# boqian-li/ETCH

Hardware: AMD Instinct MI355X
Metric: scans/s (5k pts, eq-net + 50-iter SMPL fit) (higher is better)
Workload: dtype f32 (matrix operands: 2 x fp16 planes per fp32 value, fp32 accumulate)

## Files before the change

### etch_amd/csrc/gemm.hip

```cpp
#include "common.h"
#include "split_bf16.h"
#include <cstdlib>
#include <cstring>

typedef float f32x4 __attribute__((ext_vector_type(4)));

struct GemmArgs {
    int R, K, O;
    const float* X; long ldx; const int* row_idx; int grp, p_in, p_out;
    const float* W; long ldw;
    const float* bias; const float* scale; const float* shift;
    int act;
    const float* res; long ldr; int res_mode;
    float* Y; long ldy;
};

#define G_BM 64
#define G_BN 64
#define G_BK 32
#define G_LD 40

template <bool VEC>
__device__ __forceinline__ float4 ld4_guard(const float* row, int k, int K, bool row_ok) {
    float4 v = make_float4(0.f, 0.f, 0.f, 0.f);
// ... 261 lines not shown
    l = __float_as_uint(r - __uint_as_float(m & 0xffff0000u));
}
__device__ __forceinline__ void g_split8(const float4 v0, const float4 v1, g_bf16x8 (&o)[3]) {
    const float v[8] = {v0.x, v0.y, v0.z, v0.w, v1.x, v1.y, v1.z, v1.w};
    unsigned h[8], m[8], l[8];
#pragma unroll
    for (int i = 0; i < 8; ++i) g_split(v[i], h[i], m[i], l[i]);
    typedef unsigned u32x4 __attribute__((ext_vector_type(4)));
#define G_PK(a) (u32x4){__builtin_amdgcn_perm(a[1], a[0], 0x07060302u), __builtin_amdgcn_perm(a[3], a[2], 0x07060302u), \
                        __builtin_amdgcn_perm(a[5], a[4], 0x07060302u), __builtin_amdgcn_perm(a[7], a[6], 0x07060302u)}
    const u32x4 ph = G_PK(h), pm = G_PK(m), pl = G_PK(l);
#undef G_PK
    o[0] = __builtin_bit_cast(g_bf16x8, ph); o[1] = __builtin_bit_cast(g_bf16x8, pm); o[2] = __builtin_bit_cast(g_bf16x8, pl);
}

template <int K, int SPW, int RP, bool F16 = false>
__global__ void __launch_bounds__(512) gemm_ws_split_kernel(GemmArgs a, long rows_per_block) {
    constexpr int FD_ROWS = 64, SB = K + 8, KT = K / 32, PLANE = FD_ROWS * SB;
    constexpr int NPL = F16 ? 2 : 3;
    constexpr int SG = 8 / RP;
    constexpr int RTW = (FD_ROWS / 16) / RP;
    extern __shared__ __attribute__((aligned(16))) float lds[];
    unsigned short* Xp = reinterpret_cast<unsigned short*>(lds);
    float* rsc = lds + 2 * NPL * PLANE / 2;
    float* wtab = rsc + 2 * FD_ROWS;
    const int tid = threadIdx.x, lane = tid & 63, wave = __builtin_amdgcn_readfirstlane(tid >> 6);
    const int fr = lane & 15, fg = lane >> 4;
    const int sg = wave % SG, rp = wave / SG;
    g_bf16x8 wf[KT][SPW][NPL];
    float4 wk4[SPW];
    constexpr bool EPI_REGS = KT * SPW * 12 <= 96;
    float4 bs[EPI_REGS ? SPW : 1], sc[EPI_REGS ? SPW : 1], sh[EPI_REGS ? SPW : 1];
// ... 33 lines not shown
            }
        } else {
#pragma unroll
            for (int t = 0; t < KT; ++t) {
                const float* p = a.W + (long)(o + fr) * a.ldw + 32 * t + 8 * fg;
                g_bf16x8 q3[3];
                g_split8(*reinterpret_cast<const float4*>(p), *reinterpret_cast<const float4*>(p + 4), q3);
#pragma unroll
                for (int pl = 0; pl < NPL; ++pl) wf[t][s2][pl] = q3[pl % 3];
            }
        }
        if constexpr (EPI_REGS) epi_load(o, bs[s2], sc[s2], sh[s2]);
    }
    constexpr int C4 = K / 4;
    constexpr int XL = (FD_ROWS * C4 + 511) / 512;
    const long row_lo = (long)blockIdx.x * rows_per_block, row_hi = row_lo + rows_per_block < a.R ? row_lo + rows_per_block : a.R;
    float4 xn[XL];
    static_assert(512 % C4 == 0 && (FD_ROWS * C4) % 512 == 0, "tile staging assumes whole 512-element passes");
    constexpr int RSTEP = 512 / C4;
    const int row0 = tid / C4, c0 = (tid % C4) * 4;
    auto fetch = [&](long r0) {
        const float* src = a.X + (r0 + row0) * a.ldx + c0;
#pragma unroll
        for (int h = 0; h < XL; ++h) {
            xn[h] = make_float4(0.f, 0.f, 0.f, 0.f);
            if (r0 + row0 + h * RSTEP < row_hi) xn[h] = *reinterpret_cast<const float4*>(src + (long)(h * RSTEP) * a.ldx);
        }
    };
    auto stage = [&](unsigned short* P, float* rs) {
        unsigned short* d0 = P + row0 * SB + c0;
#pragma unroll
        for (int h = 0; h < XL; ++h) {
            if constexpr (F16) {
                const int kx = etch_scale_exp(etch_group_max<C4>(etch_max4abs(xn[h], 0.f)));
                const float sx = ldexpf(1.0f, kx);
                uint2 ph, pl;
// ... 46 lines not shown
                float4 v;
                if constexpr (F16) {
                    v = make_float4(fmaf(acc[s2][0], rsv * wk4[s2].x, b_.x), fmaf(acc[s2][1], rsv * wk4[s2].y, b_.y), fmaf(acc[s2][2], rsv * wk4[s2].z, b_.z),
                                    fmaf(acc[s2][3], rsv * wk4[s2].w, b_.w));
                } else {
                    v = make_float4(acc[s2][0] + b_.x, acc[s2][1] + b_.y, acc[s2][2] + b_.z, acc[s2][3] + b_.w);
                }
                if (a.scale) { v.x = v.x * s_.x + h_.x; v.y = v.y * s_.y + h_.y; v.z = v.z * s_.z + h_.z; v.w = v.w * s_.w + h_.w; }
                float4 rs = make_float4(0.f, 0.f, 0.f, 0.f);
                if (a.res_mode != 0) rs = *reinterpret_cast<const float4*>(a.res + r * a.ldr + o);
                if (a.res_mode == 1) { v.x += rs.x; v.y += rs.y; v.z += rs.z; v.w += rs.w; }
                if (a.act == 1) { v.x = fmaxf(v.x, 0.f); v.y = fmaxf(v.y, 0.f); v.z = fmaxf(v.z, 0.f); v.w = fmaxf(v.w, 0.f); }
                else if (a.act == 2) { v.x = v.x > 0.f ? v.x : 0.01f * v.x; v.y = v.y > 0.f ? v.y : 0.01f * v.y; v.z = v.z > 0.f ? v.z : 0.01f * v.z; v.w = v.w > 0.f ? v.w : 0.01f * v.w; }
                if (a.res_mode == 2) { v.x += rs.x; v.y += rs.y; v.z += rs.z; v.w += rs.w; }
                *reinterpret_cast<float4*>(a.Y + r * a.ldy + o) = v;
            }
        }
    };
    if (row_lo >= row_hi) return;
    fetch(row_lo);
    stage(Xp, rsc);
    fetch(row_lo + FD_ROWS);
    __syncthreads();
    if constexpr (F16) {
#pragma unroll
        for (int s2 = 0; s2 < SPW; ++s2) wk4[s2] = *reinterpret_cast<const float4*>(&wtab[(wave * SPW + s2) * 16 + 4 * fg]);
    }
    int buf = 0;
    for (long r0 = row_lo; r0 < row_hi; r0 += FD_ROWS, buf ^= 1) {
        const unsigned short* P = Xp + buf * NPL * PLANE;
        row_tile(P, rp * RTW, r0, rsc + buf * FD_ROWS);
        stage(Xp + (buf ^ 1) * NPL * PLANE, rsc + (buf ^ 1) * FD_ROWS);
        if constexpr (EPI_REGS) fetch(r0 + 2 * FD_ROWS);
#pragma unroll
        for (int i = 1; i < RTW; ++i) row_tile(P, rp * RTW + i, r0, rsc + buf * FD_ROWS);
        if constexpr (!EPI_REGS) fetch(r0 + 2 * FD_ROWS);
        __syncthreads();
    }
}

template <int K, int SPW, int RP, bool F16 = false>
static int launch_ws_split(const GemmArgs& a, hipStream_t st) {
    constexpr int FD_ROWS = 64;
    const size_t lds = (size_t)2 * (F16 ? 2 : 3) * FD_ROWS * (K + 8) * 2 + (size_t)2 * FD_ROWS * sizeof(float) + (size_t)8 * SPW * 16 * sizeof(float);
    auto kern = gemm_ws_split_kernel<K, SPW, RP, F16>;
    static int per_cu = 0;
    if (per_cu == 0) {
        if (lds > 64 * 1024) {
            hipError_t e = hipFuncSetAttribute((const void*)kern, hipFuncAttributeMaxDynamicSharedMemorySize, (int)lds);
            if (e != hipSuccess) return (int)e;
        }
        int n = 0;
        if (hipOccupancyMaxActiveBlocksPerMultiprocessor(&n, (const void*)kern, 512, lds) != hipSuccess || n < 1) n = 1;
        per_cu = n;
    }
    long nb = (long)etch_cu_count() * per_cu;
    long rpb = (a.R + nb - 1) / nb;
#ifndef GEMM_WS_MIN_TILES
#define GEMM_WS_MIN_TILES 4
#endif
    if (rpb < GEMM_WS_MIN_TILES * FD_ROWS) rpb = GEMM_WS_MIN_TILES * FD_ROWS;
    rpb = (rpb + FD_ROWS - 1) / FD_ROWS * FD_ROWS;
    nb = (a.R + rpb - 1) / rpb;
    hipLaunchKernelGGL(kern, dim3((unsigned)nb), dim3(512), lds, st, a, rpb);
    ETCH_RETURN_IF_LAUNCH_FAILED();
    return ETCH_OK;
}

extern "C" int etch_linear(int R, int K, int O, const float* X, long ldx, const int* row_idx, int grp, int p_in, int p_out,
                           const float* W, long ldw, const float* bias, const float* scale, const float* shift, int act,
                           const float* res, long ldr, int res_mode, float* Y, long ldy, void* stream) {
    if (R <= 0 || O <= 0) return ETCH_OK;
    if (K <= 0) return ETCH_EINVAL;
    if ((scale == nullptr) != (shift == nullptr)) return ETCH_EINVAL;
    if (res_mode != 0 && res == nullptr) return ETCH_EINVAL;
    if (row_idx && (grp <= 0 || p_out <= 0)) return ETCH_EINVAL;
    GemmArgs a{R, K, O, X, ldx, row_idx, grp, p_in, p_out, W, ldw, bias, scale, shift, act, res, ldr, res_mode, Y, ldy};
    const bool vx = !(K & 3) && !(ldx & 3) && !((uintptr_t)X & 15);
    const bool vw = !(K & 3) && !(ldw & 3) && !((uintptr_t)W & 15);
    hipStream_t st = (hipStream_t)stream;
    if (K == 1) {
// ... 32 lines not shown
```

### etch_amd/csrc/pt.hip

```cpp
#include "common.h"

struct PtAttnParams {
    const float* p;
    const float* xq; const float* xk; const float* xv; long ldq;
    const int* idx;
    const float* W0; const float* b0; const float* s_p; const float* t_p;
    const float* W3; const float* b3;
    const float* s_w0; const float* t_w0;
    const float* W2T; const float* b2;
    const float* s_w3; const float* t_w3;
    const float* W5; const float* b5;
    const float* s_out; const float* t_out;
    float* out; long ldo;
    int n, c, ns;
};

__global__ void __launch_bounds__(128) pt_attention_kernel(PtAttnParams a) {
    extern __shared__ __attribute__((aligned(16))) float sm[];
    const int c = a.c, ns = a.ns, cs = c >> 3;
    float* s_pr = sm;
    float* s_w = s_pr + ns * c;
    float* s_h = s_w + ns * c;
    float* s_l = s_h + ns * cs;
    float* s_p3 = s_l + ns * cs;
// ... 559 lines not shown
    return v;
}
template <int NS>
__device__ __forceinline__ float pt_group_max(float v) {
    v = fmaxf(v, pt_dpp<0xB1>(v));
    v = fmaxf(v, pt_dpp<0x4E>(v));
    v = fmaxf(v, pt_dpp<0x141>(v));
    if (NS == 16) v = fmaxf(v, pt_dpp<0x140>(v));
    return v;
}

#ifndef PT_MFMA_WGS
#define PT_MFMA_WGS 4
#endif
template <int C, int NS>
__global__ void __launch_bounds__(256, PT_MFMA_WGS) pt_attention_mfma_kernel(PtAttnParams a, const float* __restrict__ W2, long ntiles) {
    constexpr int CS = C / 8;
    constexpr int MT = CS <= 16 ? 1 : CS / 16;
    constexpr int KT = C / 16;
    constexpr int PPW = 16 / NS;
    constexpr bool W2_LDS = C <= 256;
    constexpr int LDW = C + 4;
    extern __shared__ __attribute__((aligned(16))) float cst[];
    float* W3s = cst;
    float* b3s = W3s + 3 * C;
    float* scs = b3s + C;
    float* shs = scs + C;
    float* sos = shs + C;
    float* tos = sos + C;
    float* b2s = tos + C;
    float* s3s = b2s + CS;
// ... 6 lines not shown
    for (int e = tid; e < C; e += 256) {
        b3s[e] = a.b3[e]; scs[e] = a.s_w0[e]; shs[e] = a.t_w0[e];
        sos[e] = a.s_out ? a.s_out[e] : 1.f; tos[e] = a.s_out ? a.t_out[e] : 0.f;
    }
    for (int e = tid; e < CS; e += 256) { b2s[e] = a.b2[e]; s3s[e] = a.s_w3[e]; t3s[e] = a.t_w3[e]; b5s[e] = a.b5[e]; }
    for (int e = tid; e < CS * CS; e += 256) W5s[e] = a.W5[e];
    if (W2_LDS)
        for (int e = tid; e < CS * C / 4; e += 256) {
            const int row = e / (C / 4), c4 = e - row * (C / 4);
            *reinterpret_cast<float4*>(&W2s[row * LDW + c4 * 4]) = *reinterpret_cast<const float4*>(W2 + (size_t)row * C + c4 * 4);
        }
    __syncthreads();
    const int lane = tid & 63, wave = tid >> 6;
    const int fr = lane & 15, fg = lane >> 4;
    const int pw = fr / NS, jn = fr % NS;
    for (long tile = blockIdx.x; tile < ntiles; tile += gridDim.x) {
    asm volatile("" ::: "memory");
    const long base = (tile * 4 + wave) * PPW;
    const bool valid = base + pw < a.n;
    const int i = valid ? (int)(base + pw) : a.n - 1;
    const int j = a.idx[(size_t)i * NS + jn];
    float h[3];
    pt_rel_hidden(a, i, j, h);
    const float* kr = a.xk + (size_t)j * a.ldq;
    const float* qr = a.xq + (size_t)i * a.ldq;
    const float* vr = a.xv + (size_t)j * a.ldq;

    pf32x4 acc[MT];
#pragma unroll
    for (int mt = 0; mt < MT; ++mt) acc[mt] = (pf32x4){0.f, 0.f, 0.f, 0.f};
#pragma unroll 4
    for (int t = 0; t < KT; ++t) {
        const int ch0 = t * 16 + fg * 4;
        const float4 k4 = *reinterpret_cast<const float4*>(kr + ch0), q4 = *reinterpret_cast<const float4*>(qr + ch0);
        const float4 wa = *reinterpret_cast<const float4*>(W3s + ch0 * 3), wb = *reinterpret_cast<const float4*>(W3s + ch0 * 3 + 4),
// ... 68 lines not shown
                if (jn == 0 && valid) {
                    if (a.s_out) {
                        const float4 so = *reinterpret_cast<const float4*>(sos + ch0), to = *reinterpret_cast<const float4*>(tos + ch0);
                        o0 = fmaxf(o0 * so.x + to.x, 0.f); o1 = fmaxf(o1 * so.y + to.y, 0.f);
                        o2 = fmaxf(o2 * so.z + to.z, 0.f); o3 = fmaxf(o3 * so.w + to.w, 0.f);
                    }
                    *reinterpret_cast<float4*>(orow + ch0) = make_float4(o0, o1, o2, o3);
                }
            }
        }
    }
    }
}

template <int C_, int NS_>
static int launch_pt_mfma(const PtAttnParams& a, const float* W2, hipStream_t st) {
    constexpr int CS = C_ / 8, PPW = 16 / NS_;
    const size_t lds = (size_t)(8 * C_ + 4 * CS + CS * CS + (C_ <= 256 ? CS * (C_ + 4) : 0)) * sizeof(float);
    auto kern = pt_attention_mfma_kernel<C_, NS_>;
    static int per_cu = 0;
    if (per_cu == 0) {
        if (lds > 64 * 1024 && hipFuncSetAttribute((const void*)kern, hipFuncAttributeMaxDynamicSharedMemorySize, (int)lds) != hipSuccess) return ETCH_EUNSUPPORTED;
        int nb = 0;
        if (hipOccupancyMaxActiveBlocksPerMultiprocessor(&nb, (const void*)kern, 256, lds) != hipSuccess || nb < 1) nb = 1;
        per_cu = nb > 8 ? 8 : nb;
    }
    const long ntiles = ((long)a.n + 4 * PPW - 1) / (4 * PPW);
    long blocks = (long)etch_cu_count() * per_cu;
    if (blocks > ntiles) blocks = ntiles;
    hipLaunchKernelGGL(kern, dim3((unsigned)blocks), dim3(256), lds, st, a, W2, ntiles);
    ETCH_RETURN_IF_LAUNCH_FAILED();
    return ETCH_OK;
}

extern "C" int etch_pt_attention_mfma(int n, int c, int ns, const float* p, const float* xq, const float* xk, const float* xv, long ldq,
                                      const int* idx, const float* const* params, const float* W2, float* out, long ldo, void* stream) {
    if (n <= 0) return ETCH_OK;
    if ((ldq & 3) || (ldo & 3) || !W2) return ETCH_EINVAL;
    PtAttnParams a;
    fill_pt_params(a, n, c, ns, p, xq, xk, xv, ldq, idx, params, out, ldo);
    hipStream_t st = (hipStream_t)stream;
#define PT_MFMA_CASE(C_, NS_) \
    if (c == C_ && ns == NS_) return launch_pt_mfma<C_, NS_>(a, W2, st);
    PT_MFMA_CASE(64, 8) PT_MFMA_CASE(128, 8) PT_MFMA_CASE(64, 16) PT_MFMA_CASE(128, 16) PT_MFMA_CASE(256, 16) PT_MFMA_CASE(512, 16)
#undef PT_MFMA_CASE
    return ETCH_EUNSUPPORTED;
}

__global__ void __launch_bounds__(256) pt_down_gather_max_kernel(int m, int ns, int co, const float* __restrict__ ux, long ldu,
                                                                 const float* __restrict__ p, const float* __restrict__ new_p,
                                                                 const int* __restrict__ idx, const float* __restrict__ Wp,
                                                                 const float* __restrict__ scale, const float* __restrict__ shift,
                                                                 float* __restrict__ out) {
    const int c4 = co >> 2;
    const size_t total = (size_t)m * c4;
    for (size_t e = (size_t)blockIdx.x * 256 + threadIdx.x; e < total; e += (size_t)gridDim.x * 256) {
        const int i = (int)(e / c4), o0 = (int)(e - (size_t)i * c4) * 4;
        const float qx = new_p[(size_t)i * 3], qy = new_p[(size_t)i * 3 + 1], qz = new_p[(size_t)i * 3 + 2];
        float w[4][3];
#pragma unroll
        for (int u = 0; u < 4; ++u) { w[u][0] = Wp[(o0 + u) * 3]; w[u][1] = Wp[(o0 + u) * 3 + 1]; w[u][2] = Wp[(o0 + u) * 3 + 2]; }
// ... 354 lines not shown
```

### etch_amd/models/models_pointcloud.py

```python
import os

import torch
import torch.nn.init as init
from torch import nn

from .. import ops
from ..config.EPN_options import get_default_cfg
from .direction_backbones import BatchMLP, StackedMHSA
from . import pointops
from .pointnet2_utils import propagate_cl
from .pointtransformer_seg import get_pointtransformer_confidence, get_pointtransformer_magnitude
from .so3net import build_model


SUPPORTED_EPN_LAYER_NUMS = frozenset({1, 2, 3, 4})


class GT_network_equiv(nn.Module):
    def __init__(self, option=None):
        super().__init__()
        self.option = option
        model_setting_file = os.path.join(option.output_folder, "EPN_model_setting_json")
        EPN_cfg = get_default_cfg()
        EPN_cfg.model.search_radius = option.EPN_input_radius
# ... 301 lines not shown
        oh = [N * (i + 1) for i in range(B)]
        o = pointops.offsets_tensor(oh, hitpts.device)
        n_o = downsampled_offsets(oh, 4)
        n_o_t = pointops.make_offsets(n_o, hitpts.device, like=(o, 4))
        packed = hitpts.view(-1, 3)
        idx_a, idx_b = ops.fps_pair(xyz_b3n, m, packed, o, n_o_t, n_o)
        ops._FPS_READY[("vgtk", xyz_b3n.data_ptr(), int(m))] = idx_a
        ops._FPS_READY[("pointops", packed.data_ptr(), n_o_t.data_ptr())] = idx_b
        return [idx_a, idx_b, n_o_t]

    def _input_order(self, hitpts):
        if not hitpts.is_cuda:
            return None
        from .so3conv import input_xyz
        xyz = input_xyz(hitpts)
        return pointops._memo(("input_order", xyz.data_ptr(), tuple(xyz.shape)), (xyz,), lambda: ops.spatial_order(xyz))

    def _heads_streams(self):
        if not hasattr(self, "_head_streams"):
            prio = int(os.environ.get("ETCH_HEAD_STREAM_PRIORITY", "-1"))
            from ..utils.cu_streams import make_stream
            if os.environ.get("ETCH_HEAD_STREAMS", "2") == "1":
                one = make_stream("side", priority=prio)
                self._head_streams = (one, one)
            else:
                self._head_streams = (make_stream("side", priority=prio), make_stream("side", priority=prio))
        return self._head_streams

    def _forward(self, hitpts, pred_items, direction_mode, B, N):
        idx_ready = None
        if self.overlap_index_ops and hitpts.is_cuda:
# ... 74 lines not shown
```

### etch_amd/models/pointops.py

```python
import torch

from .. import ops

_knn_cache = None


def host_offsets(o):
    v = getattr(o, "_etch_host", None)
    if v is None or getattr(o, "_etch_host_version", -1) != o._version:
        v = [int(t) for t in o.tolist()]
        set_host_offsets(o, v)
    return v


def set_host_offsets(o, values):
    o._etch_host = list(values)
    o._etch_host_version = o._version
    return o


_offset_tensors = {}


def offsets_tensor(values, device):
# ... 21 lines not shown
    def __exit__(self, *a):
        global _knn_cache
        _knn_cache = self._prev


def _memo(key, keep, fn):
    if _knn_cache is None:
        return fn()
    hit = _knn_cache.get(key)
    if hit is None:
        hit = (fn(), keep)
        _knn_cache[key] = hit
    return hit[0]


def make_offsets(values, device, like=None):
    return offsets_tensor(values, device)


def furthestsampling(xyz, offset, new_offset):
    oh, noh = host_offsets(offset), host_offsets(new_offset)
    return _memo(("fps", xyz.data_ptr(), tuple(oh), tuple(noh)), (xyz,), lambda: ops.furthestsampling(xyz, offset, new_offset, oh, noh))


def gather_rows(x, idx):
    return _memo(("rows", x.data_ptr(), idx.data_ptr()), (x, idx), lambda: ops.gather_rows(x, idx))


def knnquery(nsample, xyz, new_xyz, offset, new_offset):
    if new_xyz is None:
# ... 24 lines not shown
```

### etch_amd/models/pointtransformer_seg.py

```python
import os

import torch
import torch.nn as nn

from .. import ops
from ..vgtk_so3conv import _Derived
from . import pointops


def fold_bn(bn):
    s = bn.weight.detach() / torch.sqrt(bn.running_var + bn.eps)
    return s.contiguous(), (bn.bias.detach() - bn.running_mean * s).contiguous()



def downsampled_offsets(oh, stride):
    n_o, count, prev = [], 0, 0
    for i, end in enumerate(oh):
        m = (end - prev) // stride
        if m <= 0:
            raise ValueError(f"scan {i} has {end - prev} points at a stride-{stride} TransitionDown: too few for the five-level "
                             f"Point-Transformer nets (a scan needs at least 256 points)")
        count += m
        n_o.append(count)
# ... 48 lines not shown
                      s0, t0, d(self.linear_w[2].weight).t().contiguous(), d(self.linear_w[2].bias), s3, t3,
                      d(self.linear_w[5].weight), d(self.linear_w[5].bias)]
            return wqkv, bqkv, params, (d(self.linear_w[2].weight), d(self.linear_w[2].bias), s3, t3, d(self.linear_w[5].weight), d(self.linear_w[5].bias))

        return self._d.get(ps, build)

    def forward(self, pxo, out_bn=None) -> torch.Tensor:
        p, x, o = pxo
        wqkv, bqkv, params, mlp = self._derived()
        qkv = ops.linear(x, wqkv, bias=bqkv)
        idx = pointops.knnquery(self.nsample, p, p, o, o)[0]
        allp = params + list(out_bn if out_bn is not None else (None, None))
        if self.attention_impl == "valu":
            return ops.pt_attention(p, qkv, self.out_planes, idx, allp, self.nsample)
        if self.attention_impl == "mfma" and (self.out_planes, self.nsample) in ops.PT_MFMA_SHAPES:
            return ops.pt_attention_mfma(p, qkv, self.out_planes, idx, allp, self.nsample, mlp[0])
        return ops.pt_attention_split(p, qkv, self.out_planes, idx, allp, self.nsample, *mlp)

    attention_impl = "mfma"


class TransitionDown(nn.Module):
    split_linear = True

    def __init__(self, in_planes, out_planes, stride=1, nsample=16):
        super().__init__()
        self.stride, self.nsample = stride, nsample
        if stride != 1:
            self.linear = nn.Linear(3 + in_planes, out_planes, bias=False)
            self.pool = nn.MaxPool1d(nsample)
        else:
            self.linear = nn.Linear(in_planes, out_planes, bias=False)
        self.bn = nn.BatchNorm1d(out_planes)
        self.relu = nn.ReLU(inplace=True)
# ... 248 lines not shown
```

### etch_amd/models/so3conv.py

```python
import os

import torch
import torch.nn as nn

from .. import ops
from .. import vgtk_so3conv as sptk


def input_xyz(x):
    from . import pointops
    return pointops._memo(("epn_xyz", x.data_ptr(), tuple(x.shape)), (x,), lambda: x.permute(0, 2, 1).contiguous())


_ones_cache = {}


def _occupancy_ones(b, n, na, device):
    key = (b, n, na, device.type, device.index)
    t = _ones_cache.get(key)
    if t is None:
        if len(_ones_cache) > 8:
            _ones_cache.clear()
        t = torch.ones((b, n, na, 1), dtype=torch.float32, device=device)
        torch.cuda.current_stream(device).synchronize() if device.type == "cuda" else None
# ... 53 lines not shown
        super().__init__()
        dim_in, dim_out = params["dim_in"], params["dim_out"]
        self.use_intra = params["kanchor"] > 1
        assert self.use_intra
        self.inter_conv = InterSO3ConvBlock(**params)
        self.intra_conv = IntraSO3ConvBlock(dim_out, dim_out, dropout_rate=params["dropout_rate"], activation=params["activation"])
        self.stride = params["stride"]
        self.skip_conv = nn.Conv2d(dim_in, dim_out, 1)
        self.norm = nn.InstanceNorm2d(dim_out, affine=False)
        self.emit_planes = False

    skip_on_side_stream = os.environ.get("ETCH_SKIP_STREAM", "0") == "1"
    _side = None

    fold_k1_skip = os.environ.get("ETCH_SKIP_K1_FOLD", "1") != "0"

    def _skip_branch(self, fin, sample_idx, p2):
        b, p1, na, cin = fin.shape
        w = self.skip_conv.weight.detach().view(self.skip_conv.out_channels, cin)
        bias = self.skip_conv.bias.detach()
        if cin == 1 and self.fold_k1_skip and fin.is_cuda and self.emit_planes in (False, None, "f16"):
            if getattr(fin, "_etch_constant", None) is not None:
                return ("zero",)
            f = fin.reshape(b, p1, na)
            if self.stride > 1:
                f = torch.gather(f, 1, sample_idx.long().unsqueeze(-1).expand(-1, -1, na))
            f = f.reshape(b, p2 * na)
            var, mean = torch.var_mean(f.double(), dim=1, unbiased=False, keepdim=True)
            w64, b64 = w.double().view(1, -1), bias.double().view(1, -1)
            rstd = torch.rsqrt(w64 * w64 * var + 1e-5)
            slope = (w64 * rstd).float()
            offset = ((b64 - (w64 * mean + b64)) * rstd).float()
            return ("k1", f, slope, offset)
        if self.stride > 1:
            s = ops.linear(fin.view(-1, cin), w, bias=bias, row_idx=sample_idx.contiguous(), grp=na, p_in=p1, p_out=p2, rows=b * p2 * na)
        else:
            s = ops.linear(fin.view(-1, cin), w, bias=bias)
        s = s.view(b, p2, na, -1)
        m3, r3 = ops.instnorm_stats(s)
        return s, m3, r3

    def forward(self, x, inter_idx, inter_w):
        conv = self.inter_conv.conv
        fin = x.feats_cl
        branch = None
        if self.skip_on_side_stream and fin.is_cuda and not torch.is_grad_enabled():
            main = torch.cuda.current_stream()
            if SeparableSO3ConvBlock._side is None:
# ... 95 lines not shown
```

### etch_amd/ops.py

```python
import ctypes
import math
import os

import torch

from . import _lib

_c_int, _c_float, _vp = ctypes.c_int, ctypes.c_float, ctypes.c_void_p


_raw_stream = getattr(torch._C, "_cuda_getCurrentRawStream", None)


def _stream():
    if _raw_stream is not None:
        return _vp(_raw_stream(torch.cuda.current_device()))
    return _vp(torch.cuda.current_stream().cuda_stream)


def _ptr(t):
    return _vp(t.data_ptr())


def _need(t, dtype, name):
# ... 164 lines not shown
        raise _lib.EtchHipError("x must be a float32 CUDA(HIP) tensor")
    K = x.shape[-1]
    assert x.stride(-1) == 1 and weight.shape[1] == K, (x.shape, weight.shape)
    x2 = x if x.dim() == 2 else x.reshape(-1, K)
    ldx = x2.stride(0) if x2.shape[0] > 1 else K
    R = x2.shape[0] if rows is None else rows
    O = weight.shape[0]
    if out is None:
        out = torch.empty((R, O), dtype=torch.float32, device=x.device)
    ldr = res.stride(0) if res is not None and res.dim() == 2 and res.shape[0] > 1 else O
    _lib.check(_lib.lib().etch_linear(int(R), int(K), int(O), _ptr(x2), _c_long(ldx), _optptr(row_idx), int(grp), int(p_in), int(p_out),
                                      _ptr(weight), _c_long(weight.stride(0)), _optptr(bias), _optptr(scale), _optptr(shift),
                                      ACT[act], _optptr(res), _c_long(ldr), int(res_mode), _ptr(out), _c_long(out.stride(0)), _stream()),
               "etch_linear")
    return out


def permute_weight_frag(w2):
    O, K = w2.shape
    assert O % 16 == 0 and K % 16 == 0
    return w2.reshape(O // 16, 16, K // 16, 4, 4).permute(2, 0, 3, 1, 4).contiguous().reshape(-1)


def permute_weight_frag32(w2):
    O, K = w2.shape
    assert O % 32 == 0 and K % 8 == 0
    return w2.reshape(O // 32, 32, K // 8, 2, 4).permute(2, 0, 3, 1, 4).contiguous().reshape(-1)


def inter_weight_frag(W, cin, ks=24):
# ... 429 lines not shown


def pt_attention(p, qkv, c, idx, params, ns):
    n = p.shape[0]
    out = torch.empty((n, c), dtype=torch.float32, device=p.device)
    arr = (ctypes.c_void_p * 16)(*[(0 if t is None else t.data_ptr()) for t in params])
    base = qkv.data_ptr()
    _lib.check(_lib.lib().etch_pt_attention(n, c, ns, _ptr(p), _vp(base), _vp(base + 4 * c), _vp(base + 8 * c), _c_long(qkv.stride(0)),
                                            _ptr(idx), arr, _ptr(out), _c_long(c), _stream()), "etch_pt_attention")
    return out


PT_MFMA_SHAPES = {(64, 8), (128, 8), (64, 16), (128, 16), (256, 16), (512, 16)}


def pt_attention_mfma(p, qkv, c, idx, params, ns, w2):
    n = p.shape[0]
    _need(w2, torch.float32, "w2")
    out = torch.empty((n, c), dtype=torch.float32, device=p.device)
    arr = (ctypes.c_void_p * 16)(*[(0 if t is None else t.data_ptr()) for t in params])
    base = qkv.data_ptr()
    _lib.check(_lib.lib().etch_pt_attention_mfma(n, c, ns, _ptr(p), _vp(base), _vp(base + 4 * c), _vp(base + 8 * c), _c_long(qkv.stride(0)),
                                                 _ptr(idx), arr, _ptr(w2), _ptr(out), _c_long(c), _stream()), "etch_pt_attention_mfma")
    return out


def _need_experiments(what):
    if not _lib.has_experiments():
        raise _lib.EtchHipError(f"{what} is an opt-in experiment: rebuild with ETCH_BUILD_EXPERIMENTS=1 python -m etch_amd.build")


def pt_block_k1(x, w1, s1, t1, wqkv, bqkv):
    _need_experiments("etch_pt_block_k1")
    n, c = x.shape
    assert x.stride(1) == 1 and w1.shape == (c, c) and wqkv.shape == (3 * c, c)
    qkv = torch.empty((n, 3 * c), dtype=torch.float32, device=x.device)
# ... 533 lines not shown
```

### include/etch_hip.h

```cpp
#ifndef ETCH_HIP_H
#define ETCH_HIP_H

#ifdef __cplusplus
extern "C" {
#endif


int etch_ball_query(int b, int n, int m, float radius, int nsample, const float* new_xyz, const float* xyz,
                    int* idx, void* stream);

int etch_furthest_point_sampling(int b, int n, int m, const float* xyz, int* idx, void* stream);

int etch_fps_split_workspace_bytes(int nseg, int G);
int etch_furthest_point_sampling_split(int b, int n, int m, const float* xyz, int* idx, int G, void* workspace, void* stream);
int etch_furthestsampling_split(int b, int n_max, const float* xyz, const int* offset, const int* new_offset, int* idx, int G, void* workspace,
                                void* stream);
int etch_fps_split_failed(const void* workspace, int* failed, void* stream);
int etch_fps_split_debug(unsigned spin_limit, int drop_group);
int etch_fps_fast(int enable);

int etch_gather_points(int b, int c, int n, int m, const float* points, const int* idx, float* out, void* stream);

int etch_gather_points_backward(int b, int c, int n, int m, const float* grad_out, const int* idx, float* grad_points, void* stream);

// ... 12 lines not shown
                              int* idx, float* dist, int write_sqrt, void* stream);


void knnquery_cuda_launcher(int m, int nsample, const float* xyz, const float* new_xyz, const int* offset, const int* new_offset, int* idx,
                            float* dist2);
void furthestsampling_cuda_launcher(int b, int n, const float* xyz, const int* offset, const int* new_offset, float* tmp, int* idx);
void ball_query_cuda_launcher(int b, int n, int m, float radius, int nsample, const float* new_xyz, const float* xyz, int* idx);
void furthest_point_sampling_cuda_launcher(int b, int n, int m, const float* dataset, float* temp, int* idxs);
void gather_points_forward_cuda_launcher(int b, int c, int n, int m, const float* points, const int* idx, float* out);
void gather_points_backward_cuda_launcher(int b, int c, int n, int m, const float* grad_out, const int* idx, float* grad_points);


int etch_linear(int R, int K, int O, const float* X, long ldx, const int* row_idx, int grp, int p_in, int p_out,
                const float* W, long ldw, const float* bias, const float* scale, const float* shift, int act,
                const float* res, long ldr, int res_mode, float* Y, long ldy, void* stream);


int etch_inter_so3conv(int b, int cin, int cout, int p1, int p2, int nn, float sigma, const float* xyz,
                       const float* new_xyz, const int* ball_idx, const float* feats, const float* rk, const float* W,
                       const float* Wp, const float* bias, float* out, void* stream);

int etch_inter_so3conv_ordered(int b, int cin, int cout, int p1, int p2, int nn, float sigma, const float* xyz, const float* new_xyz,
                               const int* ball_idx, const float* feats, const float* rk, const float* W, const float* Wp,
                               const float* bias, float* out, const int* order, double* stat_part, void* stream);

#ifdef ETCH_BUILD_EXPERIMENTS
int etch_inter_so3conv32(int b, int cin, int cout, int p1, int p2, int nn, float sigma, const float* xyz, const float* new_xyz,
                         const int* ball_idx, const float* feats, const float* rk, const float* Wp32, const float* bias, float* out,
                         const int* order, double* stat_part, void* stream);
#endif
// ... 79 lines not shown
int etch_so3_mean_dir_backward(long T, int A, const float* w, const float* anchors, const float* ddir, float* dw, void* stream);
int etch_weighted_segment_sum_rows(long nseg, int C, int fan, const float* src, const float* wgt, const long long* perm, const long long* seg,
                                   float* dst, void* stream);


int etch_pt_attention(int n, int c, int ns, const float* p, const float* xq, const float* xk, const float* xv, long ldq,
                      const int* idx, const float* const* params, float* out, long ldo, void* stream);

int etch_pt_attn_prep(int n, int c, int ns, const float* p, const float* xq, const float* xk, long ldq, const int* idx,
                      const float* const* params, float* w_in, void* stream);
int etch_pt_attn_aggregate(int n, int c, int ns, const float* p, const float* xv, long ldq, const int* idx, const float* logits,
                           const float* const* params, float* out, long ldo, void* stream);

int etch_pt_attention_mfma(int n, int c, int ns, const float* p, const float* xq, const float* xk, const float* xv, long ldq,
                           const int* idx, const float* const* params, const float* W2, float* out, long ldo, void* stream);

#ifdef ETCH_BUILD_EXPERIMENTS
int etch_pt_block_k1(int n, int c, const float* x, long ldx, const float* W1, const float* s1, const float* t1, const float* Wqkv,
                     const float* bqkv, float* qkv, long ldq, void* stream);
int etch_pt_block_k2(int n, int c, int ns, const float* p, const float* xq, const float* xk, const float* xv, long ldq, const int* idx,
                     const float* const* params, const float* W2, const float* const* tail, long ldx, float* out, long ldo,
                     float* qkv_next, long ldqn, void* stream);
#endif

int etch_pt_group(int m, int ns, int c, const float* p, const float* new_p, const float* x, long ldx, const int* idx,
                  float* out, long ldo, void* stream);

int etch_gather_rows(int m, int c, const float* x, long ldx, const int* idx, float* out, void* stream);

int etch_pt_down_gather_max(int m, int ns, int co, const float* ux, long ldu, const float* p, const float* new_p, const int* idx,
// ... 151 lines not shown
```

Baseline: 1049.

## Fuse skip-conv normalization stats into GEMM epilogue and spatially order PT attention

Adds a statistics variant of the warp-specialized split GEMM that accumulates per-channel sum and sum-of-squares in double inside the epilogue, followed by a small final kernel producing mean and rstd. The skip branch of the SO3 conv uses it, so a separate pass over the output to compute normalization statistics is no longer needed. Separately, the point-transformer MFMA attention kernel can follow a spatial-order schedule and split tiles into eight contiguous shares, aiming for better cache locality on neighbour gathers. Both paths are enabled by default through environment flags; they add extra double-precision work and an extra launch per stats call.

```diff
diff --git a/etch_amd/csrc/gemm.hip b/etch_amd/csrc/gemm.hip
--- a/etch_amd/csrc/gemm.hip
+++ b/etch_amd/csrc/gemm.hip
@@ -299,8 +299,10 @@
     o[0] = __builtin_bit_cast(g_bf16x8, ph); o[1] = __builtin_bit_cast(g_bf16x8, pm); o[2] = __builtin_bit_cast(g_bf16x8, pl);
 }
 
-template <int K, int SPW, int RP, bool F16 = false>
-__global__ void __launch_bounds__(512) gemm_ws_split_kernel(GemmArgs a, long rows_per_block) {
+template <int K, int SPW, int RP, bool F16 = false, bool STATS = false, bool GATHER = false>
+__global__ void __launch_bounds__(512) gemm_ws_split_kernel(GemmArgs a, long rows_per_block, long rows_per_scan, double* __restrict__ stat_part) {
+    static_assert(!STATS || (SPW == 1 && !F16), "the statistics epilogue is written for one strip per wave, three-plane operands");
+    static_assert(!GATHER || STATS, "the row map is instantiated for the skip convs only");
     constexpr int FD_ROWS = 64, SB = K + 8, KT = K / 32, PLANE = FD_ROWS * SB;
     constexpr int NPL = F16 ? 2 : 3;
     constexpr int SG = 8 / RP;
@@ -364,12 +366,41 @@
     }
     constexpr int C4 = K / 4;
     constexpr int XL = (FD_ROWS * C4 + 511) / 512;
-    const long row_lo = (long)blockIdx.x * rows_per_block, row_hi = row_lo + rows_per_block < a.R ? row_lo + rows_per_block : a.R;
+    const long scan_lo = STATS ? (long)blockIdx.y * rows_per_scan : 0, scan_hi = STATS ? scan_lo + rows_per_scan : (long)a.R;
+    const long row_lo = scan_lo + (long)blockIdx.x * rows_per_block, row_hi = row_lo + rows_per_block < scan_hi ? row_lo + rows_per_block : scan_hi;
     float4 xn[XL];
+    long gsrc[GATHER ? XL : 1];
+    double st_s[STATS ? 4 : 1], st_q[STATS ? 4 : 1];
+    if constexpr (STATS) {
+#pragma unroll
+        for (int j = 0; j < 4; ++j) st_s[j] = st_q[j] = 0.0;
+    }
     static_assert(512 % C4 == 0 && (FD_ROWS * C4) % 512 == 0, "tile staging assumes whole 512-element passes");
     constexpr int RSTEP = 512 / C4;
     const int row0 = tid / C4, c0 = (tid % C4) * 4;
+    auto lookup = [&](long r0) {
+        if constexpr (GATHER) {
+#pragma unroll
+            for (int h = 0; h < XL; ++h) {
+                const long r = r0 + row0 + h * RSTEP;
+                gsrc[h] = 0;
+                if (r < row_hi) {
+                    const int q = (int)r / a.grp;
+                    gsrc[h] = ((long)(q / a.p_out) * a.p_in + a.row_idx[q]) * a.grp + ((int)r - q * a.grp);
+                }
+            }
+        }
+    };
     auto fetch = [&](long r0) {
+        if constexpr (GATHER) {
+#pragma unroll
+            for (int h = 0; h < XL; ++h) {
+                xn[h] = make_float4(0.f, 0.f, 0.f, 0.f);
+                if (r0 + row0 + h * RSTEP < row_hi) xn[h] = *reinterpret_cast<const float4*>(a.X + gsrc[h] * a.ldx + c0);
+            }
+            lookup(r0 + FD_ROWS);
+            return;
+        }
         const float* src = a.X + (r0 + row0) * a.ldx + c0;
 #pragma unroll
         for (int h = 0; h < XL; ++h) {
@@ -446,10 +477,16 @@
                 else if (a.act == 2) { v.x = v.x > 0.f ? v.x : 0.01f * v.x; v.y = v.y > 0.f ? v.y : 0.01f * v.y; v.z = v.z > 0.f ? v.z : 0.01f * v.z; v.w = v.w > 0.f ? v.w : 0.01f * v.w; }
                 if (a.res_mode == 2) { v.x += rs.x; v.y += rs.y; v.z += rs.z; v.w += rs.w; }
                 *reinterpret_cast<float4*>(a.Y + r * a.ldy + o) = v;
+                if constexpr (STATS) {
+                    const double d0 = (double)v.x, d1 = (double)v.y, d2 = (double)v.z, d3 = (double)v.w;
+                    st_s[0] += d0; st_q[0] += d0 * d0; st_s[1] += d1; st_q[1] += d1 * d1;
+                    st_s[2] += d2; st_q[2] += d2 * d2; st_s[3] += d3; st_q[3] += d3 * d3;
+                }
             }
         }
     };
     if (row_lo >= row_hi) return;
+    lookup(row_lo);
     fetch(row_lo);
     stage(Xp, rsc);
     fetch(row_lo + FD_ROWS);
@@ -468,6 +505,45 @@
         for (int i = 1; i < RTW; ++i) row_tile(P, rp * RTW + i, r0, rsc + buf * FD_ROWS);
         if constexpr (!EPI_REGS) fetch(r0 + 2 * FD_ROWS);
         __syncthreads();
+    }
+    if constexpr (STATS) {
+        static_assert((size_t)2 * NPL * PLANE * 2 >= (size_t)512 * 4 * sizeof(double), "the tile planes hold the reduction buffer");
+        double* red = reinterpret_cast<double*>(lds);
+        const int c = tid;
+        const int csg = c >> 4, cfg = (c >> 2) & 3, cj = c & 3;
+#pragma unroll
+        for (int k = 0; k < 2; ++k) {
+#pragma unroll
+            for (int j = 0; j < 4; ++j) red[tid * 4 + j] = k == 0 ? st_s[j] : st_q[j];
+            __syncthreads();
+            if (c < 16 * SG) {
+                double t = 0.0;
+                for (int p = 0; p < RP; ++p)
+                    for (int l = 0; l < 16; ++l) t += red[(((p * SG + csg) * 64) + cfg * 16 + l) * 4 + cj];
+                stat_part[(((size_t)blockIdx.y * gridDim.x + blockIdx.x) * 2 + k) * (16 * SG) + c] = t;
+            }
+            __syncthreads();
+        }
+    }
+}
+
+__global__ void __launch_bounds__(1024) gemm_ws_stats_final_kernel(int nparts, int C, long rows, float eps, const double* __restrict__ part,
+                                                                   float* __restrict__ mean, float* __restrict__ rstd) {
+    __shared__ double red[2][1024];
+    const int b = blockIdx.x, tid = threadIdx.x;
+    const int c = tid % C, sl = tid / C, nsl = 1024 / C;
+    const double* pb = part + (size_t)b * nparts * 2 * C;
+    double s = 0.0, q = 0.0;
+    for (int k = sl; k < nparts; k += nsl) { s += pb[(size_t)k * 2 * C + c]; q += pb[(size_t)k * 2 * C + C + c]; }
+    red[0][tid] = s; red[1][tid] = q;
+    __syncthreads();
+    if (sl == 0) {
+        for (int k = 1; k < nsl; ++k) { s += red[0][k * C + c]; q += red[1][k * C + c]; }
+        const double m = s / (double)rows;
+        double var = q / (double)rows - m * m;
+        if (var < 0.0) var = 0.0;
+        mean[(size_t)b * C + c] = (float)m;
+        rstd[(size_t)b * C + c] = (float)(1.0 / sqrt(var + (double)eps));
     }
 }
 
@@ -494,9 +570,57 @@
     if (rpb < GEMM_WS_MIN_TILES * FD_ROWS) rpb = GEMM_WS_MIN_TILES * FD_ROWS;
     rpb = (rpb + FD_ROWS - 1) / FD_ROWS * FD_ROWS;
     nb = (a.R + rpb - 1) / rpb;
-    hipLaunchKernelGGL(kern, dim3((unsigned)nb), dim3(512), lds, st, a, rpb);
+    hipLaunchKernelGGL(kern, dim3((unsigned)nb), dim3(512), lds, st, a, rpb, 0L, (double*)nullptr);
     ETCH_RETURN_IF_LAUNCH_FAILED();
     return ETCH_OK;
+}
+
+#ifndef GEMM_WS_STAT_CHUNKS
+#define GEMM_WS_STAT_CHUNKS 128
+#endif
+static inline long ws_stats_rows_per_block(long rows) {
+    const long tiles = (rows + 63) / 64;
+    long tpc = (tiles + GEMM_WS_STAT_CHUNKS - 1) / GEMM_WS_STAT_CHUNKS;
+    if (tpc < GEMM_WS_MIN_TILES) tpc = GEMM_WS_MIN_TILES;
+    return tpc * 64;
+}
+static inline int ws_stats_chunks(long rows) {
+    const long rpb = ws_stats_rows_per_block(rows);
+    return (int)((rows + rpb - 1) / rpb);
+}
+
+template <int K, int SPW, int RP, bool GATHER>
+static int launch_ws_stats(const GemmArgs& a, int b, long rows, double* part, float* mean, float* rstd, hipStream_t st) {
+    constexpr int FD_ROWS = 64;
+    const size_t lds = (size_t)2 * 3 * FD_ROWS * (K + 8) * 2 + (size_t)2 * FD_ROWS * sizeof(float) + (size_t)8 * SPW * 16 * sizeof(float);
+    auto kern = gemm_ws_split_kernel<K, SPW, RP, false, true, GATHER>;
+    hipLaunchKernelGGL(kern, dim3((unsigned)ws_stats_chunks(rows), (unsigned)b), dim3(512), lds, st, a, ws_stats_rows_per_block(rows), rows, part);
+    ETCH_RETURN_IF_LAUNCH_FAILED();
+    hipLaunchKernelGGL(gemm_ws_stats_final_kernel, dim3((unsigned)b), dim3(1024), 0, st, ws_stats_chunks(rows), a.O, rows, 1e-5f, part, mean, rstd);
+    ETCH_RETURN_IF_LAUNCH_FAILED();
+    return ETCH_OK;
+}
+
+extern "C" int etch_linear_stats_chunks(int rows) { return rows > 0 ? ws_stats_chunks(rows) : 0; }
+
+extern "C" int etch_linear_stats(int b, int rows, int K, int O, const float* X, long ldx, const int* row_idx, int grp, int p_in, int p_out,
+                                 const float* W, long ldw, const float* bias, float* Y, long ldy, double* workspace, float* mean, float* rstd,
+                                 void* stream) {
+    if (b <= 0 || rows <= 0) return ETCH_OK;
+    if (!X || !W || !Y || !workspace || !mean || !rstd) return ETCH_EINVAL;
+    if (row_idx && (grp <= 0 || p_out <= 0 || p_in <= 0 || (long)p_out * grp != rows)) return ETCH_EINVAL;
+    if ((long)b * rows > 0x7fffffffL) return ETCH_EUNSUPPORTED;
+    if ((ldx & 3) || (ldw & 3) || (ldy & 3) || (((uintptr_t)X | (uintptr_t)W | (uintptr_t)Y) & 15)) return ETCH_EUNSUPPORTED;
+    GemmArgs a{(int)((long)b * rows), K, O, X, ldx, row_idx, grp, p_in, p_out, W, ldw, bias, nullptr, nullptr, 0, nullptr, 0, 0, Y, ldy};
+    hipStream_t st = (hipStream_t)stream;
+    if (row_idx) {
+        if (K == 32 && O == 64) return launch_ws_stats<32, 1, 2, true>(a, b, rows, workspace, mean, rstd, st);
+        return ETCH_EUNSUPPORTED;
+    }
+    if (K == 32 && O == 32) return launch_ws_stats<32, 1, 4, false>(a, b, rows, workspace, mean, rstd, st);
+    if (K == 32 && O == 64) return launch_ws_stats<32, 1, 2, false>(a, b, rows, workspace, mean, rstd, st);
+    if (K == 64 && O == 64) return launch_ws_stats<64, 1, 2, false>(a, b, rows, workspace, mean, rstd, st);
+    return ETCH_EUNSUPPORTED;
 }
 
 extern "C" int etch_linear(int R, int K, int O, const float* X, long ldx, const int* row_idx, int grp, int p_in, int p_out,
diff --git a/etch_amd/csrc/pt.hip b/etch_amd/csrc/pt.hip
--- a/etch_amd/csrc/pt.hip
+++ b/etch_amd/csrc/pt.hip
@@ -597,7 +597,8 @@
 #define PT_MFMA_WGS 4
 #endif
 template <int C, int NS>
-__global__ void __launch_bounds__(256, PT_MFMA_WGS) pt_attention_mfma_kernel(PtAttnParams a, const float* __restrict__ W2, long ntiles) {
+__global__ void __launch_bounds__(256, PT_MFMA_WGS) pt_attention_mfma_kernel(PtAttnParams a, const float* __restrict__ W2, long ntiles,
+                                                                             const int* __restrict__ sched, int sched_per, int shares) {
     constexpr int CS = C / 8;
     constexpr int MT = CS <= 16 ? 1 : CS / 16;
     constexpr int KT = C / 16;
@@ -634,11 +635,19 @@
     const int lane = tid & 63, wave = tid >> 6;
     const int fr = lane & 15, fg = lane >> 4;
     const int pw = fr / NS, jn = fr % NS;
-    for (long tile = blockIdx.x; tile < ntiles; tile += gridDim.x) {
+    long t0 = 0, lim = ntiles, q = blockIdx.x, step = gridDim.x;
+    if (shares) {
+        const long share = (ntiles + 7) >> 3;
+        t0 = (long)(blockIdx.x & 7) * share;
+        lim = share < ntiles - t0 ? share : ntiles - t0;
+        q = blockIdx.x >> 3; step = gridDim.x >> 3;
+    }
+    for (; q < lim; q += step) {
     asm volatile("" ::: "memory");
-    const long base = (tile * 4 + wave) * PPW;
+    const long base = ((t0 + q) * 4 + wave) * PPW;
     const bool valid = base + pw < a.n;
-    const int i = valid ? (int)(base + pw) : a.n - 1;
+    int i = valid ? (int)(base + pw) : a.n - 1;
+    if (sched) i = sched[i] + (sched_per ? i - i % sched_per : 0);
     const int j = a.idx[(size_t)i * NS + jn];
     float h[3];
     pt_rel_hidden(a, i, j, h);
@@ -737,7 +746,7 @@
 }
 
 template <int C_, int NS_>
-static int launch_pt_mfma(const PtAttnParams& a, const float* W2, hipStream_t st) {
+static int launch_pt_mfma(const PtAttnParams& a, const float* W2, const int* sched, int sched_per, int shares, hipStream_t st) {
     constexpr int CS = C_ / 8, PPW = 16 / NS_;
     const size_t lds = (size_t)(8 * C_ + 4 * CS + CS * CS + (C_ <= 256 ? CS * (C_ + 4) : 0)) * sizeof(float);
     auto kern = pt_attention_mfma_kernel<C_, NS_>;
@@ -750,24 +759,43 @@
     }
     const long ntiles = ((long)a.n + 4 * PPW - 1) / (4 * PPW);
     long blocks = (long)etch_cu_count() * per_cu;
-    if (blocks > ntiles) blocks = ntiles;
-    hipLaunchKernelGGL(kern, dim3((unsigned)blocks), dim3(256), lds, st, a, W2, ntiles);
-    ETCH_RETURN_IF_LAUNCH_FAILED();
-    return ETCH_OK;
-}
-
-extern "C" int etch_pt_attention_mfma(int n, int c, int ns, const float* p, const float* xq, const float* xk, const float* xv, long ldq,
-                                      const int* idx, const float* const* params, const float* W2, float* out, long ldo, void* stream) {
+    if (shares) {
+        long per = blocks >> 3;
+        const long share = (ntiles + 7) >> 3;
+        if (per > share) per = share;
+        if (per < 1) per = 1;
+        blocks = per * 8;
+    } else if (blocks > ntiles) blocks = ntiles;
+    hipLaunchKernelGGL(kern, dim3((unsigned)blocks), dim3(256), lds, st, a, W2, ntiles, sched, sched_per, shares);
+    ETCH_RETURN_IF_LAUNCH_FAILED();
+    return ETCH_OK;
+}
+
+static int pt_attention_mfma_dispatch(int n, int c, int ns, const float* p, const float* xq, const float* xk, const float* xv, long ldq, const int* idx,
+                                      const float* const* params, const float* W2, float* out, long ldo, const int* sched, int sched_per, int shares,
+                                      hipStream_t st) {
     if (n <= 0) return ETCH_OK;
     if ((ldq & 3) || (ldo & 3) || !W2) return ETCH_EINVAL;
     PtAttnParams a;
     fill_pt_params(a, n, c, ns, p, xq, xk, xv, ldq, idx, params, out, ldo);
-    hipStream_t st = (hipStream_t)stream;
 #define PT_MFMA_CASE(C_, NS_) \
-    if (c == C_ && ns == NS_) return launch_pt_mfma<C_, NS_>(a, W2, st);
+    if (c == C_ && ns == NS_) return launch_pt_mfma<C_, NS_>(a, W2, sched, sched_per, shares, st);
     PT_MFMA_CASE(64, 8) PT_MFMA_CASE(128, 8) PT_MFMA_CASE(64, 16) PT_MFMA_CASE(128, 16) PT_MFMA_CASE(256, 16) PT_MFMA_CASE(512, 16)
 #undef PT_MFMA_CASE
     return ETCH_EUNSUPPORTED;
+}
+
+extern "C" int etch_pt_attention_mfma(int n, int c, int ns, const float* p, const float* xq, const float* xk, const float* xv, long ldq,
+                                      const int* idx, const float* const* params, const float* W2, float* out, long ldo, void* stream) {
+    return pt_attention_mfma_dispatch(n, c, ns, p, xq, xk, xv, ldq, idx, params, W2, out, ldo, nullptr, 0, 0, (hipStream_t)stream);
+}
+
+extern "C" int etch_pt_attention_mfma_ordered(int n, int c, int ns, const float* p, const float* xq, const float* xk, const float* xv, long ldq,
+                                              const int* idx, const float* const* params, const float* W2, float* out, long ldo, const int* sched,
+                                              int sched_per, int shares, void* stream) {
+    if (sched_per < 0 || (sched && sched_per > 0 && n % sched_per)) return ETCH_EINVAL;
+    return pt_attention_mfma_dispatch(n, c, ns, p, xq, xk, xv, ldq, idx, params, W2, out, ldo, sched, sched ? sched_per : 0, shares != 0,
+                                      (hipStream_t)stream);
 }
 
 __global__ void __launch_bounds__(256) pt_down_gather_max_kernel(int m, int ns, int co, const float* __restrict__ ux, long ldu,
diff --git a/etch_amd/models/models_pointcloud.py b/etch_amd/models/models_pointcloud.py
--- a/etch_amd/models/models_pointcloud.py
+++ b/etch_amd/models/models_pointcloud.py
@@ -339,7 +339,9 @@
             return None
         from .so3conv import input_xyz
         xyz = input_xyz(hitpts)
-        return pointops._memo(("input_order", xyz.data_ptr(), tuple(xyz.shape)), (xyz,), lambda: ops.spatial_order(xyz))
+        order = pointops._memo(("input_order", xyz.data_ptr(), tuple(xyz.shape)), (xyz,), lambda: ops.spatial_order(xyz))
+        pointops.set_schedule(hitpts.view(-1, 3), order)
+        return order
 
     def _heads_streams(self):
         if not hasattr(self, "_head_streams"):
diff --git a/etch_amd/models/pointops.py b/etch_amd/models/pointops.py
--- a/etch_amd/models/pointops.py
+++ b/etch_amd/models/pointops.py
@@ -59,6 +59,18 @@
     return hit[0]
 
 
+def set_schedule(p, order):
+    if _knn_cache is not None and order is not None:
+        _knn_cache[("pt_sched", p.data_ptr(), int(p.shape[0]))] = (order, (p, order))
+
+
+def schedule(p):
+    if _knn_cache is None:
+        return None
+    hit = _knn_cache.get(("pt_sched", p.data_ptr(), int(p.shape[0])))
+    return None if hit is None else hit[0]
+
+
 def make_offsets(values, device, like=None):
     return offsets_tensor(values, device)
 
diff --git a/etch_amd/models/pointtransformer_seg.py b/etch_amd/models/pointtransformer_seg.py
--- a/etch_amd/models/pointtransformer_seg.py
+++ b/etch_amd/models/pointtransformer_seg.py
@@ -86,10 +86,13 @@
         if self.attention_impl == "valu":
             return ops.pt_attention(p, qkv, self.out_planes, idx, allp, self.nsample)
         if self.attention_impl == "mfma" and (self.out_planes, self.nsample) in ops.PT_MFMA_SHAPES:
+            if self.pt_order and self.out_planes <= 128:
+                return ops.pt_attention_mfma(p, qkv, self.out_planes, idx, allp, self.nsample, mlp[0], sched=pointops.schedule(p), shares=True)
             return ops.pt_attention_mfma(p, qkv, self.out_planes, idx, allp, self.nsample, mlp[0])
         return ops.pt_attention_split(p, qkv, self.out_planes, idx, allp, self.nsample, *mlp)
 
     attention_impl = "mfma"
+    pt_order = os.environ.get("ETCH_PT_ORDER", "1") != "0"
 
 
 class TransitionDown(nn.Module):
diff --git a/etch_amd/models/so3conv.py b/etch_amd/models/so3conv.py
--- a/etch_amd/models/so3conv.py
+++ b/etch_amd/models/so3conv.py
@@ -91,6 +91,10 @@
     _side = None
 
     fold_k1_skip = os.environ.get("ETCH_SKIP_K1_FOLD", "1") != "0"
+
+    fuse_skip_stats = os.environ.get("ETCH_SKIP_STATS", "1") != "0"
+
+    fuse_skip_stats_strided = os.environ.get("ETCH_SKIP_STATS_STRIDED", "0") == "1"
 
     def _skip_branch(self, fin, sample_idx, p2):
         b, p1, na, cin = fin.shape
@@ -109,6 +113,14 @@
             slope = (w64 * rstd).float()
             offset = ((b64 - (w64 * mean + b64)) * rstd).float()
             return ("k1", f, slope, offset)
+        strided = self.stride > 1
+        if (self.fuse_skip_stats and (self.fuse_skip_stats_strided or not strided) and fin.is_cuda and not self.training and fin.is_contiguous()
+                and (cin, w.shape[0], strided) in ops.LINEAR_STATS_SHAPES):
+            if strided:
+                s, m3, r3 = ops.linear_stats(fin, w, bias, b, p2 * na, row_idx=sample_idx.contiguous(), grp=na, p_in=p1, p_out=p2)
+            else:
+                s, m3, r3 = ops.linear_stats(fin, w, bias, b, p2 * na)
+            return s.view(b, p2, na, -1), m3, r3
         if self.stride > 1:
             s = ops.linear(fin.view(-1, cin), w, bias=bias, row_idx=sample_idx.contiguous(), grp=na, p_in=p1, p_out=p2, rows=b * p2 * na)
         else:
diff --git a/etch_amd/ops.py b/etch_amd/ops.py
--- a/etch_amd/ops.py
+++ b/etch_amd/ops.py
@@ -202,6 +202,32 @@
                                       ACT[act], _optptr(res), _c_long(ldr), int(res_mode), _ptr(out), _c_long(out.stride(0)), _stream()),
                "etch_linear")
     return out
+
+
+LINEAR_STATS_SHAPES = {(32, 32, False), (32, 64, False), (64, 64, False), (32, 64, True)}
+
+
+def linear_stats(x, weight, bias, b, rows, row_idx=None, grp=1, p_in=0, p_out=1):
+    _need(weight, torch.float32, "weight"), _need(x, torch.float32, "x")
+    K, O = x.shape[-1], weight.shape[0]
+    assert weight.shape[1] == K
+    if (K, O, row_idx is not None) not in LINEAR_STATS_SHAPES:
+        raise _lib.EtchHipError(f"etch_linear_stats is not instantiated for K = {K}, O = {O}, row map = {row_idx is not None}")
+    if row_idx is not None:
+        _need(row_idx, torch.int32, "row_idx")
+        assert row_idx.numel() == b * p_out and p_out * grp == rows
+    else:
+        assert x.numel() == b * rows * K
+    x2 = x.view(-1, K)
+    y = torch.empty((b * rows, O), dtype=torch.float32, device=x.device)
+    nch = _lib.lib().etch_linear_stats_chunks(int(rows))
+    ws = torch.empty((b * nch * 2 * O,), dtype=torch.float64, device=x.device)
+    mean = torch.empty((b, O), dtype=torch.float32, device=x.device)
+    rstd = torch.empty((b, O), dtype=torch.float32, device=x.device)
+    _lib.check(_lib.lib().etch_linear_stats(int(b), int(rows), int(K), int(O), _ptr(x2), _c_long(K), _optptr(row_idx), int(grp), int(p_in), int(p_out),
+                                            _ptr(weight), _c_long(weight.stride(0)), _optptr(bias), _ptr(y), _c_long(O), _ptr(ws), _ptr(mean),
+                                            _ptr(rstd), _stream()), "etch_linear_stats")
+    return y, mean, rstd
 
 
 def permute_weight_frag(w2):
@@ -661,12 +687,23 @@
 PT_MFMA_SHAPES = {(64, 8), (128, 8), (64, 16), (128, 16), (256, 16), (512, 16)}
 
 
-def pt_attention_mfma(p, qkv, c, idx, params, ns, w2):
+def pt_attention_mfma(p, qkv, c, idx, params, ns, w2, sched=None, shares=False):
     n = p.shape[0]
     _need(w2, torch.float32, "w2")
     out = torch.empty((n, c), dtype=torch.float32, device=p.device)
     arr = (ctypes.c_void_p * 16)(*[(0 if t is None else t.data_ptr()) for t in params])
     base = qkv.data_ptr()
+    if sched is not None or shares:
+        per = 0
+        if sched is not None:
+            _need(sched, torch.int32, "sched")
+            if sched.numel() != n or sched.dim() not in (1, 2):
+                raise ValueError(f"sched has {tuple(sched.shape)} entries for {n} points")
+            per = sched.shape[1] if sched.dim() == 2 else 0
+        _lib.check(_lib.lib().etch_pt_attention_mfma_ordered(n, c, ns, _ptr(p), _vp(base), _vp(base + 4 * c), _vp(base + 8 * c),
+                                                             _c_long(qkv.stride(0)), _ptr(idx), arr, _ptr(w2), _ptr(out), _c_long(c), _optptr(sched),
+                                                             int(per), int(bool(shares)), _stream()), "etch_pt_attention_mfma_ordered")
+        return out
     _lib.check(_lib.lib().etch_pt_attention_mfma(n, c, ns, _ptr(p), _vp(base), _vp(base + 4 * c), _vp(base + 8 * c), _c_long(qkv.stride(0)),
                                                  _ptr(idx), arr, _ptr(w2), _ptr(out), _c_long(c), _stream()), "etch_pt_attention_mfma")
     return out
diff --git a/include/etch_hip.h b/include/etch_hip.h
--- a/include/etch_hip.h
+++ b/include/etch_hip.h
@@ -50,6 +50,10 @@
 int etch_linear(int R, int K, int O, const float* X, long ldx, const int* row_idx, int grp, int p_in, int p_out,
                 const float* W, long ldw, const float* bias, const float* scale, const float* shift, int act,
                 const float* res, long ldr, int res_mode, float* Y, long ldy, void* stream);
+int etch_linear_stats(int b, int rows, int K, int O, const float* X, long ldx, const int* row_idx, int grp, int p_in, int p_out,
+                      const float* W, long ldw, const float* bias, float* Y, long ldy, double* workspace, float* mean, float* rstd,
+                      void* stream);
+int etch_linear_stats_chunks(int rows);
 
 
 int etch_inter_so3conv(int b, int cin, int cout, int p1, int p2, int nn, float sigma, const float* xyz,
@@ -159,6 +163,9 @@
 
 int etch_pt_attention_mfma(int n, int c, int ns, const float* p, const float* xq, const float* xk, const float* xv, long ldq,
                            const int* idx, const float* const* params, const float* W2, float* out, long ldo, void* stream);
+int etch_pt_attention_mfma_ordered(int n, int c, int ns, const float* p, const float* xq, const float* xk, const float* xv, long ldq,
+                                   const int* idx, const float* const* params, const float* W2, float* out, long ldo, const int* sched,
+                                   int sched_per, int shares, void* stream);
 
 #ifdef ETCH_BUILD_EXPERIMENTS
 int etch_pt_block_k1(int n, int c, const float* x, long ldx, const float* W1, const float* s1, const float* t1, const float* Wqkv,
```

New measurement: 1052, median of 6. No clear change (+0.3%).
